# louislung/DAE_RNN_News_Recommendation

Measured on AMD Instinct MI355X. Metric: training samples/sec (8000x10000 batch_all), higher is better.
Workload: dtype f16x2h

## Files before the change

dae_rnn_news_recommendation_amd/csrc/dae_api.hip:

```cpp
#include <stdarg.h>
#include <new>

#include "dae_plan.h"

namespace dae {

static thread_local char g_err[1024] = "";
thread_local LaunchTimer g_lt = {nullptr, nullptr, nullptr, 0, 0, false};
void set_error(const char* fmt, ...) {
    va_list ap;
    va_start(ap, fmt);
    vsnprintf(g_err, sizeof(g_err), fmt, ap);
    va_end(ap);
}

}

using namespace dae;

extern "C" int dae_abi_version(void) { return DAE_ABI_VERSION; }
extern "C" const char* dae_last_error(void) { return g_err; }
extern "C" int64_t dae_pad(int64_t n) { return pad128(n); }
extern "C" void dae_set_glds(int32_t nst) { set_use_glds(nst); }
extern "C" int32_t dae_gemm_w8_splits(int32_t dtype, int32_t M, int32_t N, int32_t K) { return gemm_w8_splits(dtype, M, N, K * (dtype == DAE_BF16 ? 2 : 4) / 128); }
// ... 219 lines not shown
    return nullptr;
}

extern "C" int dae_plan_set_option(dae_plan* p, const char* name, int32_t value) {
    DAE_CHECK_ARG(p && name, "plan_set_option: null argument");
    const bool on = value != 0;
    if (!strcmp(name, "encode_sparse")) p->sparse_ok = on;
    else if (!strcmp(name, "encode_bits")) p->bits_ok = on && p->cfg.dtype == DAE_BF16 && encode_bits_fits(p->Bpm, p->Hp, p->Fp, p->s_enc);
    else if (!strcmp(name, "x_bits")) p->xbits_ok = on && p->cfg.dtype == DAE_BF16;
    else if (!strcmp(name, "fused_opt")) p->fuse_opt_ok = on;
    else if (!strcmp(name, "dw_pair")) p->dw_pair_ok = on;
    else if (!strcmp(name, "dw_tr")) { DAE_CHECK_ARG(value >= -1 && value <= 1, "plan_set_option: dw_tr is -1 (auto), 0 or 1"); p->dw_tr_mode = value; p->xct_clean = false; }
    else if (!strcmp(name, "encode_w32")) p->enc_w32_ok = on && p->cfg.dtype == DAE_BF16;
    else if (!strcmp(name, "encode_w32_cols")) { DAE_CHECK_ARG(value == 64 || value == 128, "plan_set_option: encode_w32_cols is 64 or 128"); p->w32_cols = value; }
    else if (!strcmp(name, "tail")) p->tail_ok = on;
    else if (!strcmp(name, "label_with_encode")) p->label_enc_ok = on;
    else if (!strcmp(name, "ce_literal")) p->ce_literal = on;
    else if (!strcmp(name, "gather_tile")) set_gather_tile(value);
    else if (!strcmp(name, "dw_rounds")) { DAE_CHECK_ARG(value >= 1 && value <= 64, "plan_set_option: dw_rounds in 1..64"); set_use_glds(-100 - value); }
    else if (!strcmp(name, "cos_zstore")) p->cos_zstore_ok = on;
    else if (!strcmp(name, "gram_fused")) set_use_glds(on ? -20 : -19);
    else if (!strcmp(name, "decode_x3")) set_use_glds(on ? -18 : -17);
    else if (!strcmp(name, "pad_skip")) set_use_glds(on ? -12 : -11);
    else if (!strcmp(name, "miner_order")) p->miner_order_ok = on;
    else if (!strcmp(name, "miner_ranges")) p->miner_ranges_ok = on;
    else if (!strcmp(name, "miner_pack")) set_miner_pack(on);
    else if (!strcmp(name, "miner_tile")) set_miner_tile(on);
    else if (!strcmp(name, "sym_in_decode")) p->sym_ride_ok = on;
    else if (!strcmp(name, "op_scale_log2")) {
        DAE_CHECK_ARG(value >= 0 && value <= 20, "plan_set_option: op_scale_log2 in 0..20");
        DAE_CHECK_ARG(p->es == 2, "plan_set_option: op_scale_log2 applies to the 16-bit modes");
        p->op_scale = (float)(1u << value);
    }
    else if (const char* why = relayout_reason(name)) {
        DAE_CHECK_ARG(!p->bound, "plan_set_option: %s changes the %s, set it before dae_plan_bind", name, why);
        if (!strcmp(name, "x3_terms")) {
            DAE_CHECK_ARG(value >= 0 && (uint32_t)value <= X3T_ALL, "plan_set_option: x3_terms is a mask of the X3T_* bits (0..%u)", (unsigned)X3T_ALL);
            p->terms = (uint32_t)value;
        } else if (name[0] == 'x') {
            const uint32_t bit = !strcmp(name, "x3_dec_wlo") ? X3T_DEC_WLO : X3T_DH_HLO;
            p->terms = on ? (p->terms | bit) : (p->terms & ~bit);
        } else if (!strcmp(name, "decode_bn")) {
            DAE_CHECK_ARG(value == 0 || value == 64 || value == 128, "plan_set_option: decode_bn is 0 (auto), 64 or 128");
            p->dec_bn = value;
        } else if (!strcmp(name, "gram64")) {
            p->gram64_ok = on && p->gram_split;
// ... 214 lines not shown
```

dae_rnn_news_recommendation_amd/csrc/dae_gemm.hip:

```cpp
#include "dae_sym.h"
#include "dae_kernels.h"
#include "dae_label.h"
#include "dae_gemm_tile.h"

#include <type_traits>

namespace dae {

__device__ __forceinline__ bool block_to_tile(const GemmParams& p, int& tm, int& tn, int& split, int& kt0, int& kt1) {
    const int id = blockIdx.x;
    if (p.splits > 1) {
        split = id % p.splits;
        const int tile = id / p.splits;
        tn = tile % p.tiles_n;
        tm = tile / p.tiles_n;
    } else {
        split = 0;
        const int x = id & 7, l = id >> 3;
        if (p.tiles_m >= p.tiles_n) {
            const int per = (p.tiles_m + 7) >> 3;
            tm = x * per + l / p.tiles_n;
            tn = l % p.tiles_n;
            if (l >= per * p.tiles_n || tm >= p.tiles_m) return false;
        } else {
// ... 1515 lines not shown
        if constexpr (IS_COS) {
            if (pass1) {
                e.cos_part[(int64_t)(tn * 2 + w) * e.Bp + tm * BM + k] = rowok ? pyy_l[w * 128 + k] : 0.f;
                e.cos_part[(int64_t)(2 * p.tiles_n + tn * 2 + w) * e.Bp + tm * BM + k] = rowok ? pxy_l[w * 128 + k] : 0.f;
            }
        } else {
            if (e.rowloss_part) e.rowloss_part[(int64_t)(tn * 2 + w) * e.Bp + tm * BM + k] = rowok ? rowsum_l[w * 128 + k] : 0.f;
        }
        if (e.dbv_part && !pass1 && tid < 2 * BN_T) {
            const int w2 = tid / BN_T, k2 = tid % BN_T;
            e.dbv_part[(int64_t)(tm * 2 + w2) * e.Fp + tn * BN_T + k2] = colsum_l[w2 * BN_T + k2];
        }
    }
    if constexpr (!IS_COS) {
        if (e.tile_part) {
            const float v = wave64_sum_hi(wl_acc);
            if (lane == 63) pyy_l[wave] = v;
        }
        __syncthreads();
        if (e.tile_part && tid == 0) e.tile_part[tm * p.tiles_n + tn] = (pyy_l[0] + pyy_l[1]) + (pyy_l[2] + pyy_l[3]);
    }
}

static int g_nst = 2;

static int fill_params_n(GemmParams& p, int dtype, int M, int N, const GemmSegDesc* segs, int nsegs, int splits, int bn = BN, bool a_is_k_by_m = false) {
    const int es = (dtype == DAE_BF16) ? 2 : 4;
    const int kel = BKB / es;
    DAE_CHECK_ARG(dtype == DAE_BF16 || dtype == DAE_F32, "gemm: bad dtype %d", dtype);
    DAE_CHECK_ARG(M > 0 && N > 0 && M % BM == 0 && N % bn == 0, "gemm: M=%d N=%d must be positive multiples of %d / %d", M, N, BM, bn);
    DAE_CHECK_ARG(segs && nsegs >= 1 && nsegs <= GEMM_MAX_SEG, "gemm: %d K segments (1..%d)", nsegs, GEMM_MAX_SEG);
    DAE_CHECK_ARG(segs[0].K > 0, "gemm: the first K segment is empty");
    memset(p.seg, 0, sizeof(p.seg));
    memset(p.bt2, 0, sizeof(p.bt2));
    p.nseg = 0; p.ktiles_total = 0; p.epi_vec = 0; p.out_scale = 1.f;
    for (int i = 0; i < nsegs; ++i) {
        const GemmSegDesc& d = segs[i];
        DAE_CHECK_ARG(d.K >= 0 && d.K % kel == 0, "gemm: K of segment %d = %d must be a multiple of %d", i, d.K, kel);
        if (d.K == 0) continue;
        DAE_CHECK_ARG(d.A && d.Bt, "gemm: null operand in segment %d", i);
        DAE_CHECK_ARG((d.lda * es) % 16 == 0 && (d.ldb * es) % 16 == 0, "gemm: leading dimensions must be 16-byte multiples");
        DAE_CHECK_ARG(((uintptr_t)d.A % 16) == 0 && ((uintptr_t)d.Bt % 16) == 0, "gemm: operands must be 16-byte aligned");
        DAE_CHECK_ARG((uint64_t)(a_is_k_by_m ? 64 : M) * (uint64_t)(d.lda * es) < (1ull << 32) && (uint64_t)N * (uint64_t)(d.ldb * es) < (1ull << 32),
                      "gemm: an operand panel (rows x leading dimension) must stay below 4 GiB (32-bit DMA offsets)");
        p.seg[p.nseg++] = {(const char*)d.A, (const char*)d.Bt, d.lda * es, d.ldb * es, d.K / kel};
        p.ktiles_total += d.K / kel;
// ... 67 lines not shown
}
static decode_fn decode_kernel_wide(int loss, int act, bool xbits) {
#define DAE_DKW(LV, AV)                                                                                       \
    if (loss == LV && act == AV)                                                                              \
        return xbits ? gemm_decode_loss<bf16_t, LV, AV, true, BN> : gemm_decode_loss<bf16_t, LV, AV, false, BN>;
    DAE_DKW(0, 0) DAE_DKW(0, 1) DAE_DKW(0, 2) DAE_DKW(1, 0) DAE_DKW(1, 1) DAE_DKW(1, 2) DAE_DKW(2, 0) DAE_DKW(2, 1) DAE_DKW(2, 2)
#undef DAE_DKW
    return nullptr;
}
static decode_fn decode_kernel_x3(int loss, int act) {
#define DAE_DK3(LV, AV) if (loss == LV && act == AV) return gemm_decode_loss<bf16_t, LV, AV, true, DECODE_BN_BF16, false, true>;
    DAE_DK3(0, 0) DAE_DK3(0, 1) DAE_DK3(0, 2) DAE_DK3(1, 0) DAE_DK3(1, 1) DAE_DK3(1, 2) DAE_DK3(2, 0) DAE_DK3(2, 1) DAE_DK3(2, 2)
#undef DAE_DK3
    return nullptr;
}
static decode_fn decode_kernel_c2(int loss, int act, bool res) {
#define DAE_DKC(LV, AV)                                                                                       \
    if (loss == LV && act == AV)                                                                              \
        return res ? gemm_decode_loss<bf16_t, LV, AV, true, DECODE_BN_BF16, true, false, true> : gemm_decode_loss<bf16_t, LV, AV, true, DECODE_BN_BF16, false, false, true>;
    DAE_DKC(0, 0) DAE_DKC(0, 1) DAE_DKC(0, 2) DAE_DKC(1, 0) DAE_DKC(1, 1) DAE_DKC(1, 2) DAE_DKC(2, 0) DAE_DKC(2, 1) DAE_DKC(2, 2)
#undef DAE_DKC
    return nullptr;
}
static int g_decode_x3 = 1;
template <typename T> static decode_fn decode_kernel(int loss, int act) {
#define DAE_DK(LV, AV) if (loss == LV && act == AV) return gemm_decode_loss<T, LV, AV, false, (sizeof(T) == 2 ? DECODE_BN_BF16 : BN)>;
    DAE_DK(0, 0) DAE_DK(0, 1) DAE_DK(0, 2) DAE_DK(1, 0) DAE_DK(1, 1) DAE_DK(1, 2) DAE_DK(2, 0) DAE_DK(2, 1) DAE_DK(2, 2)
#undef DAE_DK
    return nullptr;
}
static int gemm_init() {
    static int rc = [] {
        const int nsts[4] = {0, 2, 3, 4};
        for (int n : nsts)
            for (int role = 0; role <= ROLE_GRAM; ++role) {
                DAE_CHECK_HIP(hipFuncSetAttribute(reinterpret_cast<const void*>(f32out_kernel<bf16_t>(n, role)),
                                                  hipFuncAttributeMaxDynamicSharedMemorySize, lds_bytes_for(n)));
                DAE_CHECK_HIP(hipFuncSetAttribute(reinterpret_cast<const void*>(f32out_kernel<float>(n, role)),
                                                  hipFuncAttributeMaxDynamicSharedMemorySize, lds_bytes_for(n)));
            }
        for (int role = 0; role <= ROLE_GRAM; ++role) {
            DAE_CHECK_HIP(hipFuncSetAttribute(reinterpret_cast<const void*>(pc_kernel<bf16_t>(role)),
                                              hipFuncAttributeMaxDynamicSharedMemorySize, lds_bytes_for(PC_NST)));
            DAE_CHECK_HIP(hipFuncSetAttribute(reinterpret_cast<const void*>(pc_kernel<float>(role)),
                                              hipFuncAttributeMaxDynamicSharedMemorySize, lds_bytes_for(PC_NST)));
        }
        {
// ... 268 lines not shown
                    rc |= (int)hipFuncSetAttribute(reinterpret_cast<const void*>(decode_kernel_x3(l, a)), hipFuncAttributeMaxDynamicSharedMemorySize,
                                                   DecGeo<DECODE_BN_BF16>::LDS_BYTES);
            return rc;
        }();
        DAE_CHECK_ARG(x3_rc == 0, "decode_loss: hipFuncSetAttribute failed");
    }
    bool c2d = false;
    if (g_decode_x3 && dtype == DAE_BF16 && e.x_bits && !wide && !x3d && !e.x2 && p.nseg == 2 && p.seg[0].A == p.seg[1].A && p.seg[0].Bt != p.seg[1].Bt &&
        p.seg[0].lda_b == p.seg[1].lda_b && p.seg[0].ldb_b == p.seg[1].ldb_b && p.seg[0].ktiles == p.seg[1].ktiles) {
        c2d = true;
        static int c2_rc = [] {
            int rc = 0;
            for (int l = 0; l < 3; ++l)
                for (int a = 0; a < 3; ++a)
                    for (int rs = 0; rs < 2; ++rs)
                        rc |= (int)hipFuncSetAttribute(reinterpret_cast<const void*>(decode_kernel_c2(l, a, rs != 0)), hipFuncAttributeMaxDynamicSharedMemorySize,
                                                       DecGeo<DECODE_BN_BF16>::LDS_BYTES);
            return rc;
        }();
        DAE_CHECK_ARG(c2_rc == 0, "decode_loss: hipFuncSetAttribute failed");
    }
    if (e.op_scale == 0.f) e.op_scale = 1.f;
    e.no_pad_skip = g_pad_skip ? 0 : 1;
    if (wide) {
        k = decode_kernel_wide(e.loss_func, e.dec_act, e.x_bits != nullptr);
        static int wide_rc = [] {
            int rc = 0;
            for (int l = 0; l < 3; ++l)
                for (int a = 0; a < 3; ++a)
                    for (int x = 0; x < 2; ++x)
                        rc |= (int)hipFuncSetAttribute(reinterpret_cast<const void*>(decode_kernel_wide(l, a, x != 0)),
                                                       hipFuncAttributeMaxDynamicSharedMemorySize, DecGeo<BN>::LDS_BYTES);
            return rc;
        }();
        DAE_CHECK_ARG(wide_rc == 0, "decode_loss: hipFuncSetAttribute failed");
    }
    if (e.delta2_2 || e.delta2_t2 || e.x2) {
        DAE_CHECK_ARG(dtype == DAE_BF16, "decode_loss: lo images of delta2 / x exist in the 16-bit split mode only");
        k = decode_kernel_res(e.loss_func, e.dec_act, e.x_bits != nullptr);
        static int res_rc = [] {
            int rc = 0;
            for (int l = 0; l < 3; ++l)
                for (int a = 0; a < 3; ++a)
                    for (int x = 0; x < 2; ++x)
                        rc |= (int)hipFuncSetAttribute(reinterpret_cast<const void*>(decode_kernel_res(l, a, x != 0)),
                                                       hipFuncAttributeMaxDynamicSharedMemorySize, DecGeo<DECODE_BN_BF16>::LDS_BYTES);
// ... 199 lines not shown
```

dae_rnn_news_recommendation_amd/csrc/dae_kernels.h:

```cpp
#pragma once
#include "dae_common.h"

namespace dae {

struct DecodeEpi {
    const float* bv;
    const void* x;
    int64_t ldx;
    const void* x2;
    const uint32_t* x_bits;
    int64_t ldxb;
    const float* cw;
    const float* cos_stats;
    float* rowloss_part;
    float* tile_part;
    float* dbv_part;
    float* cos_part;
    void* delta2; int64_t ldd;
    void* delta2_t; int64_t lddt;
    void* delta2_2; void* delta2_t2;
    int B, F, Bp, Fp;
    int dec_act, loss_func;
    int cos_pass;
    int ce_literal;
    const float* sym_G; const float* sym_scalars; void* sym_Gs; int sym_B, sym_Bp, sym_first;
    float op_scale;
    int no_pad_skip;
    float* z_io; int64_t ldz;
    int z_mode;
    int bn;
};

enum : uint32_t {
    X3T_DEC_WLO = 1u << 0,
    X3T_DEC_HLO = 1u << 1,
    X3T_DH_WLO = 1u << 2,
    X3T_DH_D2LO = 1u << 3,
    X3T_DH_HLO = 1u << 4,
    X3T_DW_D1LO = 1u << 5,
    X3T_DW_HLO = 1u << 6,
    X3T_DW_D2LO = 1u << 7,
    X3T_ENC_WLO = 1u << 8,
    X3T_ENC_XLO = 1u << 9,
    X3T_XV = 1u << 10,
    X3T_ALL = (1u << 11) - 1,
    X3T_F16_DEFAULT = X3T_DEC_WLO | X3T_DH_WLO,
};

struct LabelJob;
struct GemmSegDesc { const void* A; int64_t lda; const void* Bt; int64_t ldb; int K; };
int launch_gemm_f32out(int dtype, int M, int N, const void* A0, int64_t lda0, const void* Bt0, int64_t ldb0, int K0,
                       const void* A1, int64_t lda1, const void* Bt1, int64_t ldb1, int K1, float* C, int64_t ldc, int splits,
                       int64_t slab_stride, hipStream_t st, int role = 0, const struct LabelJob* label_job = nullptr,
                       int* label_done = nullptr, int m_valid = 0);
// ... 106 lines not shown
```

dae_rnn_news_recommendation_amd/csrc/dae_plan.h:

```cpp
#pragma once
#include "dae_kernels.h"

using namespace dae;

enum { PS_MEMSET = 0, PS_GATHER, PS_ENC_GEMM, PS_ENC_FIN, PS_LABEL, PS_GRAM, PS_MINER, PS_TRI_FIN, PS_SYM, PS_DECODE,
       PS_COS_REDUCE, PS_STATS, PS_DH_GEMM, PS_DH_FIN, PS_DW_GEMM, PS_BIAS, PS_OPT, PS_COUNT };

struct dae_plan {
    bool prof;
    hipEvent_t ev0, ev1;
    enum { PROF_POOL = 256, PROF_STEP_MAX = 48 };
    bool prof_queued;
    bool prof_stamps;
    int pev_used;
    hipEvent_t pev[PROF_POOL];
    int pev_slot[PROF_POOL / 2];
    bool ev_dw_live;
    hipEvent_t ev_dw;
    bool sym_ride_ok;
    bool miner_order_ok;
    int32_t* miner_order;
    int32_t* cls_range;
    bool miner_ranges_ok;
    double prof_ms[PS_COUNT];
    int prof_n[PS_COUNT];
    dae_config cfg;
    dae_buffers b;
    bool bound;
    int F, H, Fp, Hp, Bmax, Bpm;
    int es;
    int s_enc, s_dh, s_gram;
    uint64_t ws_bytes;
    char *x, *xc, *xct, *h_lo, *h_t, *Gs, *delta2, *delta2_t, *delta1_t, *delta1_lo, *hcat_a, *hcat_b;
    bool x3;
    char *W_lo2, *Wt_lo2, *h_t2, *delta2_2, *delta2_t2, *delta1_t2;
    char *x_2, *xct_2, *xc_2;
    int s_enc3, s_dh3;
    uint32_t terms;
    float op_scale;
    int dec_bn;
    bool dw_pair_ok;
    bool xct2_clean;
    bool enc_w32_ok;
    int w32_cols;
    bool gram_split;
    int dw_tr_mode;
    bool gram64_ok;
    float *slabs, *h_f32, *D_slabs, *G, *rowloss_part, *dbv_part, *colsum_part, *cos_part, *cos_stats, *cw, *loss_part,
        *dw_f32, *tri_scalars, *dh_extra, *rowsq_scratch, *tile_part, *zbuf;
    bool cos_zstore_ok;
    uint32_t *cnt_part, *role_cnt, *xc_bits, *x_bits;
    bool xbits_ok;
    bool xct_clean;
    bool tail_ok;
    bool fuse_opt_ok;
    bool label_enc_ok;
    bool ce_literal;
    bool sparse_ok;
    bool bits_ok;
    int32_t *dw_i32, *n_same;
    int64_t *nvalid, *dw_i64;
    uint64_t* acc;
};

static void* plan_w_lo2(const dae_plan* p) { return (p->x3 && (p->terms & X3T_DEC_WLO)) ? (void*)p->W_lo2 : nullptr; }

static int plan_dec_bn(const dae_plan* p) {
    const int def = decode_tile_n(p->cfg.dtype);
    if (p->es != 2) return def;
    const bool res = p->x3 && (p->terms & (X3T_DH_D2LO | X3T_DW_D2LO | X3T_XV));
    if (res) return def;
    if (p->dec_bn == 64 || p->dec_bn == 128) return p->dec_bn;
    const int64_t tiles64 = (int64_t)(p->Bpm / 128) * (p->Fp / 64);
    return tiles64 > 4 * 768 ? 128 : def;
}

#define RC(expr) do { if (int rc__ = (expr)) return rc__; } while (0)

static inline float plan_lr(const dae_plan* p, int adam_t) {
    float lr = p->cfg.learning_rate;
    if (p->cfg.opt == DAE_OPT_ADAM) {
        const double t = adam_t < 1 ? 1 : adam_t;
        lr = (float)((double)lr * sqrt(1.0 - pow(0.999, t)) / (1.0 - pow(0.9, t)));
    }
    return lr;
}
static inline float* plan_bias_slot(const dae_plan* p, float* slot) { return slot ? slot + (int64_t)p->Fp * p->Hp : nullptr; }
static inline int plan_opt_step(dae_plan* p, float lr, float grad_scale, int apply, void* stream, int f0 = 0, int f1 = -1) {
    return launch_opt_step(p->cfg.opt, lr, apply ? p->cfg.momentum : 0.f, grad_scale, p->b.W, p->b.bh, p->b.bv, p->b.grad, p->b.opt_s1, p->b.opt_s2, p->Fp, p->Hp,
                           p->cfg.dtype, p->b.W_lo, p->b.Wt_lo, plan_w_lo2(p), p->x3 ? p->Wt_lo2 : nullptr, apply, stream, f0, f1);
}

int plan_prof_flush(dae_plan* p);
template <class Call>
static int prof(dae_plan* p, int slot, hipStream_t st, Call&& call) {
    const bool queued = p->prof && p->prof_queued && p->pev_used + 2 <= dae_plan::PROF_POOL;
    const bool stamped = queued && p->prof_stamps && slot != PS_MEMSET;
// ... 41 lines not shown
    DW_GEMM
};
struct BatchRoute {
    int B, Bp;
    int Bk;
    bool csr_in;
    bool dense_in;
    bool copy_in;
    bool src_binary;
    EncodeRoute enc;
    bool use_xbits;
    bool own_clean;
    bool x2_clean;
    LabelPath label;
    bool x3;
    uint32_t T;
    bool x3_vals;
    float osc, oinv;
    bool explicit3;
    bool mined;
    bool fold_finalize;
    bool sym_ride;
    int dbn;
    bool is_cos;
    bool zstore;
    int s_dh;
    DwForm dw;
    bool dw_tr;
    bool tail;
    bool stats_in_tail;
    bool fuse_bias;
};
struct StepRoute : BatchRoute {
    bool backward, apply_now, ext_mine;
    bool h_only, resume;
    bool grad_out;
    bool own_opt;
    bool clear_xct, clear_xct2;
};
```

dae_rnn_news_recommendation_amd/csrc/dae_step.hip:

```cpp
#include "dae_plan.h"

static EncodeRoute encode_route(const dae_plan& p, bool csr, bool dense, bool bits_src, float scale) {
    EncodeRoute e;
    e.w32 = p.enc_w32_ok && p.cfg.dtype == DAE_BF16;
    if (csr && p.sparse_ok) e.path = ENC_SPARSE;
    else if (p.x3 && dense) e.path = ENC_X3_GEMM;
    else if (p.bits_ok && bits_src && scale == 1.0f) e.path = ENC_BITS_GEMM;
    else e.path = ENC_GEMM;
    e.splits = e.path == ENC_X3_GEMM ? p.s_enc3 : p.s_enc;
    return e;
}

struct PhaseClass { bool backward, apply_now, ext_mine; };
static PhaseClass phase_class(int phase) { return {phase != 2, phase == 0 || phase == 3, phase == 4 || phase == 5}; }

static BatchRoute batch_route(const dae_plan& p, const PhaseClass& k, int B, const int64_t* c_indptr, const float* c_values, float scale) {
    const dae_config& c = p.cfg;
    const int Fp = p.Fp, Hp = p.Hp, dt = c.dtype;
    BatchRoute r;
    memset(&r, 0, sizeof(r));
    r.B = B; r.Bp = (int)pad128(B); r.Bk = (B + 63) / 64 * 64;
    r.copy_in = c_indptr != nullptr;
    r.csr_in = c_indptr || p.b.indptr;
    r.dense_in = !r.csr_in && p.b.dense;
    r.src_binary = c_indptr ? !c_values : (p.b.indptr && !p.b.values);
    r.enc = encode_route(p, r.csr_in, r.dense_in, !c_indptr && p.b.indptr && !p.b.values, scale);
    const bool use_sparse = r.enc.path == ENC_SPARSE;
    r.use_xbits = p.xbits_ok && p.b.indptr && !p.b.values;
    r.own_clean = use_sparse && !c_indptr && r.use_xbits && encode_csr_lds_bytes(dt, r.enc.w32, p.w32_cols, Fp / 32) <= 64 * 1024;
    r.x3 = p.x3;
    r.T = p.x3 ? p.terms : 0u;
    r.x2_clean = p.x3 && (r.T & X3T_XV) && !r.use_xbits && (p.b.values || p.b.dense);
    if (p.x3) {
        uint32_t u; memcpy(&u, &scale, 4);
        r.x3_vals = (r.T & X3T_XV) && (!r.src_binary || (u & 0xffffu) != 0u || (p.b.indptr && p.b.values) || r.dense_in);
    }
    r.osc = p.es == 2 ? p.op_scale : 1.f; r.oinv = 1.f / r.osc;
    r.explicit3 = c.triplet == 3;
    const bool label_with_encode = p.tail_ok && !r.explicit3 && !k.ext_mine && r.Bp <= 1024 && p.label_enc_ok;
    const bool label_in_gather = p.tail_ok && !label_with_encode && !r.explicit3 && !k.ext_mine && !c_indptr && p.b.indptr && r.Bp <= 1024;
    r.label = k.ext_mine ? LABEL_CALLER : r.explicit3 ? LABEL_EXPLICIT : label_with_encode ? LABEL_ENCODE : (label_in_gather && !use_sparse) ? LABEL_GATHER : LABEL_OWN;
    r.mined = !k.ext_mine && (c.triplet == DAE_TRIPLET_BATCH_ALL || c.triplet == DAE_TRIPLET_BATCH_HARD);
    r.fold_finalize = (c.triplet == DAE_TRIPLET_BATCH_ALL && !c.pos_triplets_only) && !k.ext_mine;
    r.sym_ride = r.mined && k.backward && p.sym_ride_ok;
    r.dbn = plan_dec_bn(&p);
    r.is_cos = c.loss_func == DAE_LOSS_COSINE;
    r.zstore = r.is_cos && k.backward && p.cos_zstore_ok && p.zbuf;
    r.s_dh = (p.x3 && r.dense_in) ? p.s_dh3 : p.s_dh;
    const bool fuse_opt = k.backward && k.apply_now && dt == DAE_BF16 && p.fuse_opt_ok && (!p.x3 || dw_x3_fits(Fp, Hp, r.Bp));
    const bool dw_pc_grad = k.backward && !k.apply_now && dt == DAE_BF16 && p.fuse_opt_ok && (p.x3 ? dw_x3_fits(Fp, Hp, r.Bp) : dw_grad_fits(Fp, Hp, r.Bp));
    r.dw = fuse_opt ? DW_FUSED_OPT : dw_pc_grad ? DW_PC_GRAD : DW_GEMM;
    const bool dw_plain2 = !p.x3 || !(r.T & (X3T_DW_D1LO | X3T_DW_HLO | X3T_DW_D2LO | X3T_XV));
    r.dw_tr = (p.dw_tr_mode == 1 || (p.dw_tr_mode < 0 && r.dense_in)) && dt == DAE_BF16 && k.backward && (fuse_opt || dw_pc_grad) && dw_plain2 &&
              (use_sparse || r.dense_in) && (p.x3 || dw_pc_taken(Fp, Hp, r.Bk, r.Bk, !fuse_opt));
    r.tail = p.tail_ok;
    r.stats_in_tail = k.backward && r.tail;
    r.fuse_bias = k.apply_now;
    return r;
}

static StepRoute step_route(const dae_plan& p, const dae_step& s) {
    const PhaseClass k = phase_class(s.phase);
    StepRoute r;
    memset(&r, 0, sizeof(r));
    static_cast<BatchRoute&>(r) = batch_route(p, k, s.B, s.c_indptr, s.c_values, s.scale);
    r.backward = k.backward; r.apply_now = k.apply_now; r.ext_mine = k.ext_mine;
    r.h_only = s.phase == 4; r.resume = s.phase == 5;
    r.grad_out = s.phase != 3;
// ... 176 lines not shown
                                 p->cnt_part, p->G, p->role_cnt, order, st, cls));
    else
        PROF(PS_MINER, dae_triplet_batch_hard(p->D_slabs, p->s_gram, dslab, Bp, s->labels, B, Bp, p->loss_part, p->cnt_part, p->dw_i32, p->G,
                                  stream));
    if (!r.fold_finalize)
        PROF(PS_TRI_FIN, dae_triplet_finalize(c.triplet, c.pos_triplets_only, B, Bp, c.alpha, p->loss_part, p->cnt_part, p->nvalid,
                                p->dw_i32, p->role_cnt, p->dw_f32, p->cw, p->tri_scalars, stream));
    if (r.backward && !r.sym_ride) PROF(PS_SYM, launch_sym_scale(p->G, B, Bp, p->tri_scalars, dt, p->Gs, r.osc, st));
    return 0;
}

static int stage_decode(dae_plan* p, const dae_step*, const StepRoute& r, hipStream_t st) {
    const dae_config& c = p->cfg;
    const int B = r.B, Bp = r.Bp, Fp = p->Fp, Hp = p->Hp, dt = c.dtype;
    const uint32_t T = r.T;
    const bool backward = r.backward;
    DecodeEpi e;
    memset(&e, 0, sizeof(e));
    e.bv = p->b.bv; e.x = p->x; e.ldx = Fp; e.x_bits = r.use_xbits ? p->x_bits : nullptr; e.ldxb = Fp / 32; e.cw = p->cw; e.cos_stats = r.is_cos ? p->cos_stats : nullptr;
    e.rowloss_part = r.is_cos ? p->rowloss_part : nullptr; e.tile_part = r.is_cos ? nullptr : p->tile_part;
    e.dbv_part = backward ? p->dbv_part : nullptr; e.cos_part = p->cos_part;
    e.delta2 = backward ? p->delta2 : nullptr; e.ldd = Fp; e.delta2_t = (backward && !r.dw_tr) ? p->delta2_t : nullptr; e.lddt = p->Bpm;
    e.B = B; e.F = p->F; e.Bp = Bp; e.Fp = Fp; e.dec_act = c.dec_act; e.loss_func = c.loss_func; e.ce_literal = p->ce_literal ? 1 : 0;
    e.op_scale = r.osc; e.bn = r.dbn;
    if (r.sym_ride) { e.sym_G = p->G; e.sym_scalars = p->tri_scalars; e.sym_Gs = p->Gs; e.sym_B = B; e.sym_Bp = Bp; }
    GemmSegDesc dsegs[3] = {{p->h_lo, Hp, p->b.W_lo, Hp, Hp}, {nullptr, 0, nullptr, 0, 0}, {nullptr, 0, nullptr, 0, 0}};
    int ndseg = 1;
    if (r.x3) {
        dsegs[0] = {p->hcat_a, 3 * (int64_t)Hp, p->b.W_lo, Hp, Hp};
        dsegs[1] = {p->hcat_a, 3 * (int64_t)Hp, p->W_lo2, Hp, (T & X3T_DEC_WLO) ? Hp : 0};
        dsegs[2] = {p->hcat_a + (size_t)2 * Hp * 2, 3 * (int64_t)Hp, p->b.W_lo, Hp, (T & X3T_DEC_HLO) ? Hp : 0};
        ndseg = 3;
        if (backward) { e.delta2_2 = (T & X3T_DH_D2LO) ? p->delta2_2 : nullptr; e.delta2_t2 = (T & X3T_DW_D2LO) ? p->delta2_t2 : nullptr; }
        if (r.x2_clean) e.x2 = p->x_2;
    }
    if (!r.is_cos) {
        e.cos_pass = 0;
        PROF(PS_DECODE, launch_decode_loss_n(dt, Bp, Fp, dsegs, ndseg, e, st));
        return 0;
    }
    e.cos_pass = 1;
    if (r.zstore) { e.z_io = p->zbuf; e.ldz = Fp; e.z_mode = 1; }
    PROF(PS_DECODE, launch_decode_loss_n(dt, Bp, Fp, dsegs, ndseg, e, st));
    if (r.zstore) e.z_mode = 2;
    PROF(PS_COS_REDUCE, dae_cos_reduce(p->cos_part, 2 * Fp / r.dbn, B, Bp, p->cos_stats, p->rowloss_part, (void*)st));
    e.sym_G = nullptr;
    if (backward) { e.cos_pass = 2; PROF(PS_DECODE, launch_decode_loss_n(dt, Bp, Fp, dsegs, ndseg, e, st)); }
    return 0;
}

static StatsArgs stats_args(const dae_plan* p, const dae_step* s, const StepRoute& r) {
    const dae_config& c = p->cfg;
    return StatsArgs{r.is_cos ? p->rowloss_part : nullptr, 1, r.is_cos ? nullptr : p->tile_part, (r.Bp / 128) * (p->Fp / r.dbn), p->cw, r.B, r.Bp,
                     c.triplet == 3 ? DAE_TRIPLET_BATCH_HARD : c.triplet, c.alpha, p->tri_scalars,
                     (c.triplet == DAE_TRIPLET_BATCH_ALL && !r.ext_mine) ? p->nvalid : nullptr, s->stats, r.fold_finalize ? p->loss_part : nullptr,
                     r.fold_finalize ? p->cnt_part : nullptr};
}
static int stage_stats(dae_plan* p, const dae_step* s, const StepRoute& r, hipStream_t st) {
    const StatsArgs sa = stats_args(p, s, r);
    PROF(PS_STATS, dae_step_stats(sa.rowloss_part, sa.n_col_waves, sa.tile_part, sa.n_tiles, sa.cw, r.B, r.Bp, sa.triplet, sa.alpha, sa.tri_scalars,
                                  sa.nvalid, sa.loss_part, sa.cnt_part, s->stats, (void*)st));
    return 0;
}

static int stage_dh(dae_plan* p, const dae_step*, const StepRoute& r, hipStream_t st) {
    const int B = r.B, Bp = r.Bp, Fp = p->Fp, Hp = p->Hp, ldB = p->Bpm, dt = p->cfg.dtype, Bk = r.Bk;
    const uint32_t T = r.T;
    const bool mined = r.mined;
    const int64_t slab = (int64_t)Bp * Hp;
    if (r.x3) {
        const GemmSegDesc hs[5] = {{p->delta2, Fp, p->b.Wt_lo, Fp, Fp}, {p->delta2, Fp, p->Wt_lo2, Fp, (T & X3T_DH_WLO) ? Fp : 0},
                                   {p->delta2_2, Fp, p->b.Wt_lo, Fp, (T & X3T_DH_D2LO) ? Fp : 0},
                                   {p->Gs, Bp, p->h_t, ldB, mined ? Bk : 0}, {p->Gs, Bp, p->h_t2, ldB, (mined && (T & X3T_DH_HLO)) ? Bk : 0}};
        PROF(PS_DH_GEMM, launch_gemm_f32out_n(dt, Bp, Hp, hs, 5, p->slabs, Hp, r.s_dh, slab, st, GEMM_ROLE_DH, nullptr, nullptr, 1.f, B));
    } else {
        PROF(PS_DH_GEMM, launch_gemm_f32out(dt, Bp, Hp, p->delta2, Fp, p->b.Wt_lo, Fp, Fp, mined ? p->Gs : nullptr, Bp, mined ? p->h_t : nullptr, ldB,
// ... 28 lines not shown
        }
        if (r.x3) {
            oe.W_lo2 = (T & X3T_DEC_WLO) ? p->W_lo2 : nullptr; oe.Wt_lo2 = p->Wt_lo2;
            PROF(PS_DW_GEMM, launch_dw_opt_n(Fp, Hp, ws, 6, oe, st, p->dw_pair_ok, r.dw_tr));
        } else {
            PROF(PS_DW_GEMM, launch_dw_opt(Fp, Hp, ws[0].A, ws[0].lda, ws[0].Bt, ws[0].ldb, Bk, ws[3].A, ws[3].lda, ws[3].Bt, ws[3].ldb, Bk, oe, st, r.dw_tr));
        }
    } else if (r.x3) {
        PROF(PS_DW_GEMM, launch_gemm_f32out_n(dt, Fp, Hp, ws, 6, p->b.grad, Hp, 1, 0, st, GEMM_ROLE_DW, nullptr, nullptr, r.oinv));
    } else {
        const GemmSegDesc ws2[2] = {ws[0], ws[3]};
        PROF(PS_DW_GEMM, launch_gemm_f32out_n(dt, Fp, Hp, ws2, 2, p->b.grad, Hp, 1, 0, st, GEMM_ROLE_DW, nullptr, nullptr, r.oinv));
        if (!r.apply_now && dt == DAE_BF16 && p->b.grad_lo) RC(launch_cast_bf16(p->b.grad, p->b.grad_lo, (int64_t)Fp * Hp, st));
    }
    p->ev_dw_live = false;
    if (p->ev_dw) { DAE_CHECK_HIP(hipEventRecord(p->ev_dw, st)); p->ev_dw_live = true; }
    return 0;
}

static int stage_tail(dae_plan* p, const dae_step* s, const StepRoute& r, hipStream_t st) {
    const dae_config& c = p->cfg;
    const int B = r.B, Bp = r.Bp, F = p->F, H = p->H, Fp = p->Fp, Hp = p->Hp;
    float* g_bh = p->b.grad + (int64_t)Fp * Hp;
    const BiasArgs ba{p->dbv_part, 2 * Bp / 128, p->colsum_part, Bp / 32, p->b.bh, H, Hp, F, Fp, c.enc_act, g_bh, g_bh + Hp,
                      r.fuse_bias ? 1 : 0, c.opt, plan_lr(p, s->adam_t), c.momentum, s->grad_scale, p->b.bv,
                      plan_bias_slot(p, p->b.opt_s1), plan_bias_slot(p, p->b.opt_s2)};
    if (r.tail) {
        const StatsArgs sa = stats_args(p, s, r);
        const ClearArgs ca{s->c_indptr ? s->c_indptr : p->b.indptr, s->c_indptr ? s->c_indices : p->b.indices,
                           (s->c_indptr && s->c_row_idx) ? s->c_row_idx : s->row_idx, B, F, p->xct, r.dw_tr ? (int64_t)Fp : (int64_t)p->Bpm, p->es,
                           r.x3_vals ? p->xct_2 : nullptr, r.dw_tr ? 1 : 0};
        PROF(PS_BIAS, launch_step_tail(ba, &sa, r.csr_in ? &ca : nullptr, st));
        if (r.csr_in) { p->xct_clean = true; if (r.x3_vals) p->xct2_clean = true; }
    } else {
        PROF(PS_BIAS, dae_bias_grads(ba.dbv_part, ba.n_row_waves, ba.colsum_part, ba.n_row_blocks, ba.bh, ba.H, ba.Hp, ba.F, ba.Fp, ba.enc_act, ba.dbh, ba.dbv,
                                     ba.apply, ba.opt, ba.lr, ba.mom, ba.gscale, ba.bv, ba.s1b, ba.s2b, (void*)st));
    }
    if (r.own_opt) PROF(PS_OPT, plan_opt_step(p, plan_lr(p, s->adam_t), s->grad_scale, 2, (void*)st));
    return 0;
}

static int train_step_body(dae_plan* p, const dae_step* s, void* stream) {
    DAE_CHECK_ARG(p && p->bound && s, "train_step: plan not bound / null step");
    DAE_CHECK_ARG(s->row_idx && s->B > 0 && s->B <= p->Bmax, "train_step: batch %d outside (0, %d]", s ? s->B : -1, p->Bmax);
    const dae_config& c = p->cfg;
    const bool explicit3 = (c.triplet == 3);
    DAE_CHECK_ARG(c.triplet == DAE_TRIPLET_NONE || explicit3 || s->labels, "train_step: labels required for triplet mining");
// ... 44 lines not shown
```

Baseline: 4.293 million.

## Add 160-row decode GEMM tile so the decode grid fits one round

```diff
diff --git a/dae_rnn_news_recommendation_amd/csrc/dae_api.hip b/dae_rnn_news_recommendation_amd/csrc/dae_api.hip
--- a/dae_rnn_news_recommendation_amd/csrc/dae_api.hip
+++ b/dae_rnn_news_recommendation_amd/csrc/dae_api.hip
@@ -265,6 +265,12 @@
     else if (!strcmp(name, "gram_fused")) set_use_glds(on ? -20 : -19);
     else if (!strcmp(name, "decode_x3")) set_use_glds(on ? -18 : -17);
     else if (!strcmp(name, "pad_skip")) set_use_glds(on ? -12 : -11);
+    else if (!strcmp(name, "decode_bm")) {
+        DAE_CHECK_ARG(value == 0 || value == 128 || value == 160, "plan_set_option: decode_bm is 0 (auto), 128 or 160");
+        DAE_CHECK_ARG(value != 160 || plan_dec_bm160_form(p, p->xbits_ok),
+                      "plan_set_option: decode_bm = 160 needs the three-term 16-bit decode with a bit image of x (f16x2h on a binary CSR train set; no cosine loss, no lo images of delta2 / x, decode_bn 64)");
+        p->dec_bm = value;
+    }
     else if (!strcmp(name, "miner_order")) p->miner_order_ok = on;
     else if (!strcmp(name, "miner_ranges")) p->miner_ranges_ok = on;
     else if (!strcmp(name, "miner_pack")) set_miner_pack(on);
diff --git a/dae_rnn_news_recommendation_amd/csrc/dae_gemm.hip b/dae_rnn_news_recommendation_amd/csrc/dae_gemm.hip
--- a/dae_rnn_news_recommendation_amd/csrc/dae_gemm.hip
+++ b/dae_rnn_news_recommendation_amd/csrc/dae_gemm.hip
@@ -1561,6 +1561,327 @@
     }
 }
 
+struct Dec160 {
+    static constexpr int ROWS = 160, COLS = 128, MT = ROWS / 32;
+    static constexpr int A_BYTES = ROWS * BKB;
+    static constexpr int STAGE = A_BYTES + COLS * BKB;
+    static constexpr int LOOP_BYTES = 2 * STAGE;
+    static constexpr int P0 = COLS * 2 + 16;
+    static constexpr int P1 = ROWS * 2 + 16;
+    static constexpr int R_BYTES = ROWS * P0 > COLS * P1 ? ROWS * P0 : COLS * P1;
+    static constexpr int AUX_FLOATS = ROWS + COLS + 4 * ROWS + COLS + 4;
+    static constexpr int EPI_BYTES = R_BYTES + AUX_FLOATS * 4;
+    static_assert(EPI_BYTES <= LOOP_BYTES, "the epilogue reuses the stage ring");
+    static constexpr int XB_OFF = LOOP_BYTES;
+    static constexpr int XB_PIECES = ROWS * (COLS / 32) / 64;
+    static constexpr int LDS_BYTES = XB_OFF + ROWS * (COLS / 32) * 4;
+    static_assert(LDS_BYTES <= 80 * 1024, "two workgroups per CU");
+    static_assert(P0 % 16 == 0 && P1 % 16 == 0, "16-byte pieces of the staged tiles");
+};
+template <int OFF> __device__ __forceinline__ i32x4 lds_read_b128_at(uint32_t addr) {
+    static_assert(OFF >= 0 && OFF < 65536 && OFF % 16 == 0, "a 16-bit immediate");
+    i32x4 v;
+    asm volatile("ds_read_b128 %0, %1 offset:%2" : "=&v"(v) : "v"(addr), "n"(OFF));
+    return v;
+}
+template <int KK, int SLOT> __device__ __forceinline__ void dec160_read(uint32_t a_row, uint32_t b_row, uint32_t so0, i32x4 (&fa)[5], i32x4 (&fb)[1]) {
+    static_assert(frag_slot(KK, 0) == (frag_slot(0, 0) ^ (KK << 5)) && frag_slot(KK, 63) == (frag_slot(0, 63) ^ (KK << 5)), "k step as an XOR on the slot offset");
+    uint32_t a, b;
+    if constexpr (KK == 0) { a = a_row + so0; b = b_row + so0; }
+    else {
+        asm volatile("v_xad_u32 %0, %1, %2, %3" : "=v"(a) : "v"(so0), "s"(KK << 5), "v"(a_row));
+        asm volatile("v_xad_u32 %0, %1, %2, %3" : "=v"(b) : "v"(so0), "s"(KK << 5), "v"(b_row));
+    }
+    fa[0] = lds_read_b128_at<SLOT>(a);
+    fa[1] = lds_read_b128_at<SLOT + FRAG_BLOCK>(a);
+    fa[2] = lds_read_b128_at<SLOT + 2 * FRAG_BLOCK>(a);
+    fa[3] = lds_read_b128_at<SLOT + 3 * FRAG_BLOCK>(a);
+    fa[4] = lds_read_b128_at<SLOT + 4 * FRAG_BLOCK>(a);
+    fb[0] = lds_read_b128_at<SLOT>(b);
+}
+__device__ __forceinline__ void mainloop_160_x3(const GemmParams& p, int tm, int tn, int Bp, char* lds, f32x16 (&acc)[5][1]) {
+    using T = bf16_t;
+    constexpr int STAGE = Dec160::STAGE, A_BYTES = Dec160::A_BYTES;
+    const int lane = threadIdx.x & 63;
+    const int wave = __builtin_amdgcn_readfirstlane(threadIdx.x >> 6);
+    zero_acc(acc);
+    const int nk = p.seg[0].ktiles;
+    if (nk <= 0) return;
+    static_assert(piece_slot(4, 9) == piece_slot(0, 9) && piece_slot(17, 60) == piece_slot(1, 60) && PIECE_ROWS == 8, "the piece swizzle repeats every 16 rows");
+    const uint32_t lda = (uint32_t)p.seg[0].lda_b, ldb = (uint32_t)p.seg[0].ldb_b;
+    const uint32_t slot16 = (uint32_t)(piece_slot(wave, lane) << 4);
+    const uint32_t vA = (uint32_t)(lane >> 3) * lda + slot16, vB = (uint32_t)(lane >> 3) * ldb + slot16;
+    int64_t rA[5], rB[4];
+#pragma unroll
+    for (int i = 0; i < 5; ++i) rA[i] = (int64_t)min(tm * Dec160::ROWS + (4 * i + wave) * PIECE_ROWS, Bp - PIECE_ROWS) * lda;
+#pragma unroll
+    for (int i = 0; i < 4; ++i) rB[i] = (int64_t)(tn * Dec160::COLS + (4 * i + wave) * PIECE_ROWS) * ldb;
+    auto dma = [&](char* slot, const char* gA, const char* gB) {
+#pragma unroll
+        for (int i = 0; i < 5; ++i) glds_piece<4>(i, wave, gA + rA[i] + vA, slot);
+#pragma unroll
+        for (int i = 0; i < 4; ++i) glds_piece<4>(i, wave, gB + rB[i] + vB, slot + A_BYTES);
+    };
+    const uint32_t lbase = lds_addr(lds);
+    const uint32_t a_row = lbase + frag_row(0, lane), b_row = lbase + A_BYTES + frag_row(wave * 32, lane);
+    const uint32_t so0 = frag_slot(0, lane);
+    const char *gAh = p.seg[0].A, *gBh = p.seg[0].Bt, *gAl = p.seg[2].A, *gBl = p.seg[1].Bt;
+    dma(lds, gAh, gBh);
+    dma(lds + STAGE, gAl, gBl);
+    for (int i = 0; i < nk; ++i) {
+        const bool more = i + 1 < nk;
+        wait_vm<9>();
+        __builtin_amdgcn_s_barrier();
+        asm volatile("" ::: "memory");
+        i32x4 fah[4][5], fbh[4][1];
+        dec160_read<0, 0>(a_row, b_row, so0, fah[0], fbh[0]);
+        dec160_read<1, 0>(a_row, b_row, so0, fah[1], fbh[1]);
+        mma_group<T, 6>(fah[0], fbh[0], acc);
+        __builtin_amdgcn_sched_barrier(0);
+        dec160_read<2, 0>(a_row, b_row, so0, fah[2], fbh[2]);
+        mma_group<T, 6>(fah[1], fbh[1], acc);
+        __builtin_amdgcn_sched_barrier(0);
+        dec160_read<3, 0>(a_row, b_row, so0, fah[3], fbh[3]);
+        mma_group<T, 6>(fah[2], fbh[2], acc);
+        __builtin_amdgcn_sched_barrier(0);
+        wait_lgkm<0>();
+        __builtin_amdgcn_sched_barrier(0);
+        __builtin_amdgcn_s_barrier();
+        asm volatile("" ::: "memory");
+        if (more) {
+            gAh += BKB; gBh += BKB;
+            dma(lds, gAh, gBh);
+        }
+        __builtin_amdgcn_sched_barrier(0);
+        mma_block<T>(fah[3], fbh[3], acc);
+        __builtin_amdgcn_sched_barrier(0);
+        if (more) wait_vm<9>();
+        else wait_vm<0>();
+        __builtin_amdgcn_s_barrier();
+        asm volatile("" ::: "memory");
+        i32x4 fal[2][5], fbl[2][1];
+        dec160_read<0, STAGE>(a_row, b_row, so0, fal[0], fbl[0]);
+        dec160_read<1, STAGE>(a_row, b_row, so0, fal[1], fbl[1]);
+        mma_group<T, 6>(fah[0], fbl[0], acc); mma_block<T>(fal[0], fbh[0], acc);
+        __builtin_amdgcn_sched_barrier(0);
+        dec160_read<2, STAGE>(a_row, b_row, so0, fal[0], fbl[0]);
+        mma_group<T, 6>(fah[1], fbl[1], acc); mma_block<T>(fal[1], fbh[1], acc);
+        __builtin_amdgcn_sched_barrier(0);
+        dec160_read<3, STAGE>(a_row, b_row, so0, fal[1], fbl[1]);
+        mma_group<T, 6>(fah[2], fbl[0], acc); mma_block<T>(fal[0], fbh[2], acc);
+        __builtin_amdgcn_sched_barrier(0);
+        wait_lgkm<0>();
+        __builtin_amdgcn_sched_barrier(0);
+        __builtin_amdgcn_s_barrier();
+        asm volatile("" ::: "memory");
+        if (more) {
+            gAl += BKB; gBl += BKB;
+            dma(lds + STAGE, gAl, gBl);
+        }
+        __builtin_amdgcn_sched_barrier(0);
+        mma_block<T>(fah[3], fbl[1], acc); mma_block<T>(fal[1], fbh[3], acc);
+        __builtin_amdgcn_sched_barrier(0);
+    }
+}
+
+template <int LOSS, int ACT>
+__global__ __launch_bounds__(GEMM_THREADS, 2) void gemm_decode_loss_160(GemmParams p, DecodeEpi e) {
+    static_assert(LOSS != DAE_LOSS_COSINE, "the cosine passes stay on the 128-row kernels");
+    using T = bf16_t;
+    using Geo = Dec160;
+    constexpr int ROWS = Geo::ROWS, COLS = Geo::COLS, MT = Geo::MT, P0 = Geo::P0, P1 = Geo::P1, WPR = COLS / 32;
+    extern __shared__ __attribute__((aligned(16))) char lds[];
+    if (e.sym_G && (int)blockIdx.x >= e.sym_first) {
+        const int t = (int)blockIdx.x - e.sym_first, nt = e.sym_Bp / 64;
+        sym_scale_tile<T>(e.sym_G, e.sym_B, e.sym_Bp, e.sym_scalars, reinterpret_cast<T*>(e.sym_Gs), t % nt, t / nt,
+                          reinterpret_cast<float(*)[65]>(lds), e.op_scale);
+        return;
+    }
+    int tm, tn, split, kt0, kt1;
+    if (!block_to_tile(p, tm, tn, split, kt0, kt1)) return;
+    const int tid = threadIdx.x;
+    const int lane = tid & 63, wave = tid >> 6;
+    const int g = lane >> 5, c = lane & 31;
+    const int row0 = tm * ROWS;
+    T* D2 = reinterpret_cast<T*>(e.delta2);
+    T* D2T = reinterpret_cast<T*>(e.delta2_t);
+
+    uint32_t* xb_l = reinterpret_cast<uint32_t*>(lds + Geo::XB_OFF);
+    {
+        const int wv = __builtin_amdgcn_readfirstlane(wave);
+#pragma unroll
+        for (int i = 0; i < (Geo::XB_PIECES + 3) / 4; ++i) {
+            const int piece = 4 * i + wv;
+            if (piece < Geo::XB_PIECES) {
+                const int idx = piece * 64 + lane, row = min(row0 + (idx >> 2), e.Bp - 1);
+                __builtin_amdgcn_global_load_lds((const __attribute__((address_space(1))) void*)(e.x_bits + (int64_t)row * e.ldxb + tn * WPR + (idx & 3)),
+                                                 (__attribute__((address_space(3))) void*)(xb_l + piece * 64), 4, 0, 0);
+            }
+        }
+    }
+
+    f32x16 acc[MT][1];
+    const int vblk = e.no_pad_skip ? MT : max(0, min(MT, (e.B - row0 + 31) >> 5));
+    if (vblk > 0) mainloop_160_x3(p, tm, tn, e.Bp, lds, acc);
+    else zero_acc(acc);
+    wait_vm<0>();
+    __syncthreads();
+
+    char* R = lds;
+    float* aux = reinterpret_cast<float*>(lds + Geo::R_BYTES);
+    float* cw_l = aux;
+    float* bv_l = aux + ROWS;
+    float* rowsum_l = bv_l + COLS;
+    float* colsum_l = rowsum_l + 4 * ROWS;
+    float* wl_l = colsum_l + COLS;
+    if (tid < ROWS) cw_l[tid] = (row0 + tid) < e.Bp ? e.cw[row0 + tid] : 0.f;
+    if (tid < COLS) bv_l[tid] = (tn * COLS + tid) < e.F ? e.bv[tn * COLS + tid] : 0.f;
+    __syncthreads();
+
+    const int lcol0 = wave * 32 + c;
+    const int lrow0 = 4 * g;
+    const float eps = 1e-16f;
+    const float cm = (tn * COLS + lcol0) < e.F ? 1.f : 0.f;
+    const float bvv = bv_l[lcol0];
+    float colsum = 0.f;
+    char* r0_lane = R + lrow0 * P0 + lcol0 * 2;
+    char* r1_lane = R + lcol0 * P1 + lrow0 * 2;
+    const bool want_rows = e.rowloss_part != nullptr;
+    const float osc = e.op_scale;
+    float wl_acc = 0.f;
+    uint32_t tp[MT * 4][2];
+    auto epi_block = [&](auto MTV, auto R4, auto FASTV) {
+        constexpr int mt = decltype(MTV)::value, r4 = decltype(R4)::value;
+        constexpr bool FAST = decltype(FASTV)::value;
+        constexpr int rloc = acc_row(mt, 4 * r4, 0);
+        float d2v[4];
+#pragma unroll
+        for (int q = 0; q < 4; ++q) {
+            const int lrow = lrow0 + rloc + q;
+            const float cwi = cw_l[lrow];
+            const float z = acc[mt][0][r4 * 4 + q] + bvv;
+            const float x = (float)((xb_l[lrow * WPR + wave] >> c) & 1u);
+            float rl, d2;
+            if constexpr (FAST) {
+                const float en = __builtin_amdgcn_exp2f(-fabsf(z) * kLog2e);
+                const float op = 1.0f + en;
+                const float rr = __builtin_amdgcn_rcpf(op);
+                const float yv = z >= 0.f ? rr : en * rr;
+                const float l = kLn2 * __builtin_amdgcn_logf(op) + fmaxf(z, 0.f) - x * z;
+                d2 = (cwi * cm) * (yv - x);
+                rl = cm * l;
+            } else {
+                const float y = act_fwd<ACT>(z);
+                float l, dy;
+                if constexpr (LOSS == DAE_LOSS_CROSS_ENTROPY) {
+                    const float a = y + eps, b = (1.0f - y) + eps;
+                    const float la = __builtin_amdgcn_logf(a), lb = __builtin_amdgcn_logf(b);
+                    l = -kLn2 * (x * la + (1.0f - x) * lb);
+                    dy = (1.0f - x) * __builtin_amdgcn_rcpf(b) - x * __builtin_amdgcn_rcpf(a);
+                } else {
+                    const float d = x - y;
+                    l = d * d;
+                    dy = -2.0f * d;
+                }
+                d2 = (cwi * cm) * dy * act_bwd<ACT>(y);
+                rl = cm * l;
+            }
+            colsum += d2;
+            const float d2s = sat16(d2 * osc);
+            d2v[q] = d2s;
+            *reinterpret_cast<bf16_t*>(r0_lane + (rloc + q) * P0) = f2bf_hw(d2s);
+            wl_acc += cwi * rl;
+            if (want_rows) {
+                rl = half32_sum_hi(rl);
+                if (c == 31) rowsum_l[wave * ROWS + lrow] = rl;
+            }
+        }
+        tp[mt * 4 + r4][0] = f2bf_pack_hw(d2v[0], d2v[1]);
+        tp[mt * 4 + r4][1] = f2bf_pack_hw(d2v[2], d2v[3]);
+    };
+    auto zero_block = [&](auto MTV) {
+        constexpr int mt = decltype(MTV)::value;
+#pragma unroll
+        for (int r4 = 0; r4 < 4; ++r4) {
+            const int rloc = acc_row(mt, 4 * r4, 0);
+#pragma unroll
+            for (int q = 0; q < 4; ++q) {
+                *reinterpret_cast<bf16_t*>(r0_lane + (rloc + q) * P0) = (bf16_t)0;
+                if (want_rows && c == 31) rowsum_l[wave * ROWS + lrow0 + rloc + q] = 0.f;
+            }
+            tp[mt * 4 + r4][0] = 0u; tp[mt * 4 + r4][1] = 0u;
+        }
+    };
+#define DAE_EPI160_ROWS(MTV, FV)                                                                                           \
+    if (MTV < vblk) {                                                                                                      \
+    epi_block(std::integral_constant<int, MTV>{}, std::integral_constant<int, 0>{}, std::integral_constant<bool, FV>{});   \
+    epi_block(std::integral_constant<int, MTV>{}, std::integral_constant<int, 1>{}, std::integral_constant<bool, FV>{});   \
+    epi_block(std::integral_constant<int, MTV>{}, std::integral_constant<int, 2>{}, std::integral_constant<bool, FV>{});   \
+    epi_block(std::integral_constant<int, MTV>{}, std::integral_constant<int, 3>{}, std::integral_constant<bool, FV>{});   \
+    } else zero_block(std::integral_constant<int, MTV>{});
+#define DAE_EPI160_ALL(FV) DAE_EPI160_ROWS(0, FV) DAE_EPI160_ROWS(1, FV) DAE_EPI160_ROWS(2, FV) DAE_EPI160_ROWS(3, FV) DAE_EPI160_ROWS(4, FV)
+    bool fast = false;
+    if constexpr (LOSS == DAE_LOSS_CROSS_ENTROPY && ACT == DAE_ACT_SIGMOID) {
+        float zmax = 0.f;
+#pragma unroll
+        for (int mt = 0; mt < MT; ++mt)
+#pragma unroll
+            for (int r = 0; r < 16; ++r) zmax = fmaxf(zmax, fabsf(acc[mt][0][r] + bvv));
+        fast = __builtin_amdgcn_ballot_w64(!(zmax < CE_FAST_ZMAX)) == 0ull && !e.ce_literal;
+    }
+    if (fast) {
+        if constexpr (LOSS == DAE_LOSS_CROSS_ENTROPY && ACT == DAE_ACT_SIGMOID) { DAE_EPI160_ALL(true) }
+    } else {
+        DAE_EPI160_ALL(false)
+    }
+#undef DAE_EPI160_ALL
+#undef DAE_EPI160_ROWS
+    {
+        const float v = colsum + __shfl_xor(colsum, 32, 64);
+        if (g == 0) colsum_l[lcol0] = v;
+    }
+    if (e.tile_part) {
+        const float v = wave64_sum_hi(wl_acc);
+        if (lane == 63) wl_l[wave] = v;
+    }
+    __syncthreads();
+
+    if (D2) {
+#pragma unroll
+        for (int i = 0; i < ROWS * (COLS / 8) / GEMM_THREADS; ++i) {
+            const int ch = tid + GEMM_THREADS * i, row = ch >> 4, c16 = ch & 15;
+            if (row0 + row < e.Bp)
+                *reinterpret_cast<i32x4*>(D2 + (int64_t)(row0 + row) * e.ldd + tn * COLS + c16 * 8) = *reinterpret_cast<const i32x4*>(R + row * P0 + c16 * 16);
+        }
+    }
+    if (D2T) {
+        __syncthreads();
+#pragma unroll
+        for (int mt = 0; mt < MT; ++mt)
+#pragma unroll
+            for (int r4 = 0; r4 < 4; ++r4) {
+                uint2 v; v.x = tp[mt * 4 + r4][0]; v.y = tp[mt * 4 + r4][1];
+                *reinterpret_cast<uint2*>(r1_lane + acc_row(mt, 4 * r4, 0) * 2) = v;
+            }
+        __syncthreads();
+        static_assert(COLS * (ROWS / 8) % GEMM_THREADS == 0, "whole rounds of 16-byte pieces");
+#pragma unroll
+        for (int i = 0; i < COLS * (ROWS / 8) / GEMM_THREADS; ++i) {
+            const int ch = tid + GEMM_THREADS * i, row = ch / (ROWS / 8), c16 = ch % (ROWS / 8);
+            if (row0 + c16 * 8 < e.Bp)
+                *reinterpret_cast<i32x4*>(D2T + (int64_t)(tn * COLS + row) * e.lddt + row0 + c16 * 8) = *reinterpret_cast<const i32x4*>(R + row * P1 + c16 * 16);
+        }
+    }
+    if (want_rows) {
+        for (int i = tid; i < 4 * ROWS; i += GEMM_THREADS) {
+            const int w = i / ROWS, k = i % ROWS;
+            if (row0 + k < e.Bp) e.rowloss_part[(int64_t)(tn * 4 + w) * e.Bp + row0 + k] = (row0 + k) < e.B ? rowsum_l[i] : 0.f;
+        }
+    }
+    if (e.dbv_part && tid < COLS) e.dbv_part[(int64_t)tm * e.Fp + tn * COLS + tid] = colsum_l[tid];
+    if (e.tile_part && tid == 0) e.tile_part[tm * p.tiles_n + tn] = (wl_l[0] + wl_l[1]) + (wl_l[2] + wl_l[3]);
+}
+
 static int g_nst = 2;
 
 static int fill_params_n(GemmParams& p, int dtype, int M, int N, const GemmSegDesc* segs, int nsegs, int splits, int bn = BN, bool a_is_k_by_m = false) {
@@ -1674,7 +1995,22 @@
 #undef DAE_DKC
     return nullptr;
 }
+static decode_fn decode_kernel_160(int loss, int act) {
+#define DAE_DK160(LV, AV) if (loss == LV && act == AV) return gemm_decode_loss_160<LV, AV>;
+    DAE_DK160(0, 0) DAE_DK160(0, 1) DAE_DK160(0, 2) DAE_DK160(1, 0) DAE_DK160(1, 1) DAE_DK160(1, 2)
+#undef DAE_DK160
+    return nullptr;
+}
 static int g_decode_x3 = 1;
+bool decode_bm160_form(int dtype, int bn, bool x_bits, bool three_terms, bool lo_images, int loss_func, int Fp) {
+    return g_decode_x3 && dtype == DAE_BF16 && bn == DECODE_BN_BF16 && x_bits && three_terms && !lo_images && loss_func != DAE_LOSS_COSINE && Fp % Dec160::COLS == 0;
+}
+static int gemm_init();
+bool decode_bm160_one_round(int Bp, int Fp) {
+    if (gemm_init() || g_cus <= 0) return false;
+    const int t160 = ((Bp + Dec160::ROWS - 1) / Dec160::ROWS) * (Fp / Dec160::COLS), t64 = (Bp / BM) * (Fp / DECODE_BN_BF16);
+    return t160 <= 2 * g_cus && t64 > 3 * g_cus;
+}
 template <typename T> static decode_fn decode_kernel(int loss, int act) {
 #define DAE_DK(LV, AV) if (loss == LV && act == AV) return gemm_decode_loss<T, LV, AV, false, (sizeof(T) == 2 ? DECODE_BN_BF16 : BN)>;
     DAE_DK(0, 0) DAE_DK(0, 1) DAE_DK(0, 2) DAE_DK(1, 0) DAE_DK(1, 1) DAE_DK(1, 2) DAE_DK(2, 0) DAE_DK(2, 1) DAE_DK(2, 2)
@@ -1989,6 +2325,31 @@
     }
     if (e.op_scale == 0.f) e.op_scale = 1.f;
     e.no_pad_skip = g_pad_skip ? 0 : 1;
+    DAE_CHECK_ARG(e.bm == 0 || e.bm == BM || e.bm == Dec160::ROWS, "decode_loss: tile height %d (0, 128 or 160)", e.bm);
+    if (e.bm == Dec160::ROWS) {
+        DAE_CHECK_ARG(x3d && e.loss_func != DAE_LOSS_COSINE && !e.z_io && Fp % Dec160::COLS == 0 && e.Bp == Bp && e.Fp == Fp && e.ldxb >= Fp / 32,
+                      "decode_loss: the 160-row tile exists for the three-term 16-bit decode with a bit image of x (no cosine loss, no lo images)");
+        static int rc160 = [] {
+            int rc = 0;
+            for (int l = 0; l < 2; ++l)
+                for (int a = 0; a < 3; ++a)
+                    rc |= (int)hipFuncSetAttribute(reinterpret_cast<const void*>(decode_kernel_160(l, a)), hipFuncAttributeMaxDynamicSharedMemorySize, Dec160::LDS_BYTES);
+            return rc;
+        }();
+        DAE_CHECK_ARG(rc160 == 0, "decode_loss: hipFuncSetAttribute failed");
+        GemmParams q = p;
+        q.tiles_m = (Bp + Dec160::ROWS - 1) / Dec160::ROWS; q.tiles_n = Fp / Dec160::COLS;
+        int nblocks = grid_blocks(q);
+        if (e.sym_G) {
+            DAE_CHECK_ARG(e.sym_scalars && e.sym_Gs && e.sym_Bp % 64 == 0 && e.sym_B <= e.sym_Bp, "decode_loss: bad sym_scale rider");
+            e.sym_first = nblocks;
+            nblocks += (e.sym_Bp / 64) * (e.sym_Bp / 64);
+        }
+        static_assert(Dec160::LDS_BYTES >= 64 * 65 * 4, "rider tile must fit the decode LDS");
+        DAE_LAUNCH(decode_kernel_160(e.loss_func, e.dec_act), dim3(nblocks), dim3(GEMM_THREADS), Dec160::LDS_BYTES, st, q, e);
+        DAE_CHECK_LAUNCH();
+        return 0;
+    }
     if (wide) {
         k = decode_kernel_wide(e.loss_func, e.dec_act, e.x_bits != nullptr);
         static int wide_rc = [] {
diff --git a/dae_rnn_news_recommendation_amd/csrc/dae_kernels.h b/dae_rnn_news_recommendation_amd/csrc/dae_kernels.h
--- a/dae_rnn_news_recommendation_amd/csrc/dae_kernels.h
+++ b/dae_rnn_news_recommendation_amd/csrc/dae_kernels.h
@@ -29,7 +29,10 @@
     float* z_io; int64_t ldz;
     int z_mode;
     int bn;
+    int bm;
 };
+bool decode_bm160_form(int dtype, int bn, bool x_bits, bool three_terms, bool lo_images, int loss_func, int Fp);
+bool decode_bm160_one_round(int Bp, int Fp);
 
 enum : uint32_t {
     X3T_DEC_WLO = 1u << 0,
diff --git a/dae_rnn_news_recommendation_amd/csrc/dae_plan.h b/dae_rnn_news_recommendation_amd/csrc/dae_plan.h
--- a/dae_rnn_news_recommendation_amd/csrc/dae_plan.h
+++ b/dae_rnn_news_recommendation_amd/csrc/dae_plan.h
@@ -39,6 +39,7 @@
     uint32_t terms;
     float op_scale;
     int dec_bn;
+    int dec_bm;
     bool dw_pair_ok;
     bool xct2_clean;
     bool enc_w32_ok;
@@ -73,6 +74,12 @@
     if (p->dec_bn == 64 || p->dec_bn == 128) return p->dec_bn;
     const int64_t tiles64 = (int64_t)(p->Bpm / 128) * (p->Fp / 64);
     return tiles64 > 4 * 768 ? 128 : def;
+}
+
+static bool plan_dec_bm160_form(const dae_plan* p, bool x_bits) {
+    const uint32_t T = p->x3 ? p->terms : 0u;
+    return decode_bm160_form(p->cfg.dtype, plan_dec_bn(p), x_bits, (T & X3T_DEC_WLO) && (T & X3T_DEC_HLO), (T & (X3T_DH_D2LO | X3T_DW_D2LO | X3T_XV)) != 0,
+                             p->cfg.loss_func, p->Fp);
 }
 
 #define RC(expr) do { if (int rc__ = (expr)) return rc__; } while (0)
@@ -160,6 +167,7 @@
     bool fold_finalize;
     bool sym_ride;
     int dbn;
+    int dbm;
     bool is_cos;
     bool zstore;
     int s_dh;
diff --git a/dae_rnn_news_recommendation_amd/csrc/dae_step.hip b/dae_rnn_news_recommendation_amd/csrc/dae_step.hip
--- a/dae_rnn_news_recommendation_amd/csrc/dae_step.hip
+++ b/dae_rnn_news_recommendation_amd/csrc/dae_step.hip
@@ -44,6 +44,7 @@
     r.fold_finalize = (c.triplet == DAE_TRIPLET_BATCH_ALL && !c.pos_triplets_only) && !k.ext_mine;
     r.sym_ride = r.mined && k.backward && p.sym_ride_ok;
     r.dbn = plan_dec_bn(&p);
+    r.dbm = (p.dec_bm == 160 || (p.dec_bm == 0 && plan_dec_bm160_form(&p, r.use_xbits) && decode_bm160_one_round(r.Bp, Fp))) ? 160 : 128;
     r.is_cos = c.loss_func == DAE_LOSS_COSINE;
     r.zstore = r.is_cos && k.backward && p.cos_zstore_ok && p.zbuf;
     r.s_dh = (p.x3 && r.dense_in) ? p.s_dh3 : p.s_dh;
@@ -266,7 +267,7 @@
     e.dbv_part = backward ? p->dbv_part : nullptr; e.cos_part = p->cos_part;
     e.delta2 = backward ? p->delta2 : nullptr; e.ldd = Fp; e.delta2_t = (backward && !r.dw_tr) ? p->delta2_t : nullptr; e.lddt = p->Bpm;
     e.B = B; e.F = p->F; e.Bp = Bp; e.Fp = Fp; e.dec_act = c.dec_act; e.loss_func = c.loss_func; e.ce_literal = p->ce_literal ? 1 : 0;
-    e.op_scale = r.osc; e.bn = r.dbn;
+    e.op_scale = r.osc; e.bn = r.dbn; e.bm = r.dbm;
     if (r.sym_ride) { e.sym_G = p->G; e.sym_scalars = p->tri_scalars; e.sym_Gs = p->Gs; e.sym_B = B; e.sym_Bp = Bp; }
     GemmSegDesc dsegs[3] = {{p->h_lo, Hp, p->b.W_lo, Hp, Hp}, {nullptr, 0, nullptr, 0, 0}, {nullptr, 0, nullptr, 0, 0}};
     int ndseg = 1;
@@ -295,7 +296,7 @@
 
 static StatsArgs stats_args(const dae_plan* p, const dae_step* s, const StepRoute& r) {
     const dae_config& c = p->cfg;
-    return StatsArgs{r.is_cos ? p->rowloss_part : nullptr, 1, r.is_cos ? nullptr : p->tile_part, (r.Bp / 128) * (p->Fp / r.dbn), p->cw, r.B, r.Bp,
+    return StatsArgs{r.is_cos ? p->rowloss_part : nullptr, 1, r.is_cos ? nullptr : p->tile_part, r.dbm == 160 ? ((r.Bp + 159) / 160) * (p->Fp / 128) : (r.Bp / 128) * (p->Fp / r.dbn), p->cw, r.B, r.Bp,
                      c.triplet == 3 ? DAE_TRIPLET_BATCH_HARD : c.triplet, c.alpha, p->tri_scalars,
                      (c.triplet == DAE_TRIPLET_BATCH_ALL && !r.ext_mine) ? p->nvalid : nullptr, s->stats, r.fold_finalize ? p->loss_part : nullptr,
                      r.fold_finalize ? p->cnt_part : nullptr};
@@ -370,7 +371,7 @@
     const dae_config& c = p->cfg;
     const int B = r.B, Bp = r.Bp, F = p->F, H = p->H, Fp = p->Fp, Hp = p->Hp;
     float* g_bh = p->b.grad + (int64_t)Fp * Hp;
-    const BiasArgs ba{p->dbv_part, 2 * Bp / 128, p->colsum_part, Bp / 32, p->b.bh, H, Hp, F, Fp, c.enc_act, g_bh, g_bh + Hp,
+    const BiasArgs ba{p->dbv_part, r.dbm == 160 ? (Bp + 159) / 160 : 2 * Bp / 128, p->colsum_part, Bp / 32, p->b.bh, H, Hp, F, Fp, c.enc_act, g_bh, g_bh + Hp,
                       r.fuse_bias ? 1 : 0, c.opt, plan_lr(p, s->adam_t), c.momentum, s->grad_scale, p->b.bv,
                       plan_bias_slot(p, p->b.opt_s1), plan_bias_slot(p, p->b.opt_s2)};
     if (r.tail) {
```

After: 4.337 million, median of 6. 1.01x the previous value.
